# Snoworday/instance-segmentation-attention

Hardware: AMD Instinct MI355X
Metric: images/sec @256x256 bs=16 per GPU (higher is better)
Workload: dtype bf16; 1 GPU; train.py step fwd+bwd+update 256x256 bs=16/GPU (bf16); global_batch=16, parallelism=dp1, launch=hipGraph replay

## Files before the change

include/isa_kernels.h:

```cpp
#ifndef ISA_KERNELS_H
#define ISA_KERNELS_H

#include <stdint.h>

#ifdef __cplusplus
extern "C" {
#endif

enum { ISA_F32 = 0, ISA_BF16 = 1,
       ISA_F16 = 2 };
enum { ISA_ACT_NONE = 0, ISA_ACT_RELU = 1, ISA_ACT_RELU6 = 2, ISA_ACT_LEAKY = 3, ISA_ACT_TANH = 4 };
enum { ISA_STAT_REPLICAS = 8 };
enum { ISA_OK = 0, ISA_EINVAL = -1, ISA_EALIGN = -2, ISA_EDTYPE = -3, ISA_ELAUNCH = -4, ISA_ENOMEM = -5 };

enum { ISA_IN_1X1 = 0,
       ISA_IN_3X3 = 1,
       ISA_IN_GATHER2 = 2 };
enum { ISA_OUT_PLAIN = 0,
       ISA_OUT_SHUFFLE2 = 1 };

typedef struct isa_tensor {
    void*   data;
    int32_t n, h, w;
    int32_t c;
// ... 114 lines not shown
    float count; int32_t c;
} isa_bn_upd;
int isa_bn_running_update(const isa_bn_upd* upd, int32_t n, float momentum, void* stream);
int isa_bn_bwd_reduce(const isa_tensor* dt, const isa_tensor* y, const float* scale,
                      const float* shift, const float* mean, const float* invstd, int32_t act,
                      const float* bscale, float* red, void* stream);
int isa_bn_bwd_apply(const isa_tensor* dt, const isa_tensor* y, const float* scale,
                     const float* shift, const float* mean, const float* invstd, int32_t act,
                     const float* bscale, const float* gamma, const float* red, float count,
                     int32_t train, const isa_tensor* dy, float* dgamma, float* dbeta,
                     void* stream);

int isa_affine_act_res(const isa_tensor* x, const isa_pro* pro, const isa_tensor* res,
                       const isa_tensor* res2, const float* oscale, const isa_tensor* out,
                       void* stream);
int isa_axpy(const isa_tensor* src, const isa_tensor* dst, float alpha, int32_t accumulate,
             void* stream);

int isa_avgpool2(const isa_tensor* x, const isa_tensor* y, void* stream);
int isa_avgpool2_bwd(const isa_tensor* dy, const isa_tensor* dx, int32_t accumulate, void* stream);
int isa_avgpool3(const isa_tensor* x, const isa_tensor* mask, const isa_tensor* y, int32_t accumulate,
                 void* stream);

int isa_chan_mean(const isa_tensor* x, const isa_pro* pro, float* out, void* stream);
int isa_se_fc(const float* mean, const float* w1, const float* b1, const float* w2,
              const float* b2, int32_t n, int32_t c, int32_t hidden, float* hid, float* gate,
              void* stream);
int isa_chan_argmax(const isa_tensor* x, const isa_tensor* y, void* stream);

int isa_mask_dot(const isa_tensor* x, const float* m, const float* w, const float* bias,
// ... 266 lines not shown
```

instance-segmentation-attention_amd/csrc/dwconv.hip:

```cpp
#include "common.hpp"
#include <type_traits>

namespace {

constexpr int TH = 8, TW = 32, CB = 32, PS = 36;
constexpr int HALO = (TH + 2) * (TW + 2);

struct Dw2Params {
    const void* x; const void* w; const float* bias; void* y; const void* dy;
    int n, h, w_, c, ldx, ldy, ldd, wld;
    ProDev pro;
    float* stats; int accumulate;
    int tiles_x, tiles_y; long ntiles;
    float* ws; int csrc;
    int G;
    FinDev fin;
};


struct ProRegs { float sc[8], sh[8], bs[8]; };

template <bool HAS_PRO>
__device__ __forceinline__ void load_pro(const Dw2Params& p, ProRegs& r, int c0, int b) {
#pragma unroll
// ... 514 lines not shown
}

template <typename T>
int launch_fwd2(Dw2Params& p, bool has_pro, hipStream_t s) {
    p.tiles_x = (p.w_ + TW - 1) / TW; p.tiles_y = (p.h + TH - 1) / TH;
    p.ntiles = (long)p.n * p.tiles_x * p.tiles_y;
    if (p.ntiles * p.G >= (1L << 31)) return ISA_EINVAL;
    const int ncb = (p.c + CB - 1) / CB;
    long gx = (256L * (sizeof(T) == 2 ? 1 : 3)) / ncb;
    if (gx < 1) gx = 1;
    if (gx > p.ntiles * p.G) gx = p.ntiles * p.G;
    gx = group_grid(gx, p.G);
    dim3 grid((unsigned)gx, ncb);
    if (p.accumulate) return has_pro ? ISA_EINVAL : launch_fwd2_inst<T, false, ISA_ACT_NONE, true>(p, grid, s);
    if (has_pro && p.pro.act == ISA_ACT_RELU6) return launch_fwd2_inst<T, true, ISA_ACT_RELU6>(p, grid, s);
    if (has_pro) return launch_fwd2_inst<T, true, ACT_RT>(p, grid, s);
    return launch_fwd2_inst<T, false, ISA_ACT_NONE>(p, grid, s);
}

template <typename T>
int launch_wg2(Dw2Params& p, bool has_pro, long ws_floats, isa_slab_arena* sa, const isa_pro* fin, hipStream_t s) {
    p.tiles_x = (p.w_ + TW - 1) / TW; p.tiles_y = (p.h + TH - 1) / TH;
    p.ntiles = (long)p.n * p.tiles_x * p.tiles_y;
    const int ncb = (p.c + CB - 1) / CB;
    long gx = (256L * 2) / ncb;
    if (gx < 1) gx = 1;
    if (gx > p.ntiles * p.G) gx = p.ntiles * p.G;
    if (int rc = defer_ws(sa, &p.ws, &ws_floats)) return rc;
    const long ws_cap = ws_floats / (10L * CB * ncb);
    if (ws_cap < p.G) return sa ? ISA_ENOMEM : ISA_EINVAL;
// ... 21 lines not shown
    int accumulate, tiles_x, tiles_y; long ntiles; float* ws; int csrc; float* dw;
    const void* addend; int lda;
    int G;
};


template <typename T> struct dd_stride { static constexpr int v = 36; };
template <> struct dd_stride<bf16_t> { static constexpr int v = 40; };

constexpr int DW_BIAS = 4;
template <typename T, int YACT, int XMODE_, bool DB, bool EPI>
__global__ __launch_bounds__(DB ? 512 : 256) __attribute__((amdgpu_waves_per_eu(2, 2))) void dw_bn_bwd_kernel(FusedParams p) {
    constexpr int XMODE = XMODE_ & 3;
    constexpr bool BIAS = (XMODE_ & DW_BIAS) != 0;
    constexpr int PSD = dd_stride<T>::v;
    constexpr int XACT = XMODE == 1 ? ISA_ACT_RELU6 : (XMODE == 0 ? ISA_ACT_NONE : ACT_RT);
    constexpr int NBUF = DB ? 2 : 1;
    constexpr int NTHR = DB ? 512 : 256;
    constexpr int TILE_ELEMS = HALO * PSD;
    extern __shared__ __attribute__((aligned(16))) float sm[];
    T* xt_base = reinterpret_cast<T*>(sm);
    T* dt_base = xt_base + NBUF * TILE_ELEMS;
    float* wts = reinterpret_cast<float*>(dt_base + NBUF * TILE_ELEMS);
    float* cst = wts + 9 * CB;
    float* red = cst + 10 * CB;
    f32x4* dbl = reinterpret_cast<f32x4*>(red + 12 * CB);
    constexpr bool DB_LDS = BIAS && XMODE != 0;
    const int tid = threadIdx.x;
    const int ltid = tid & 255;
    const bool loader = DB && tid >= 256;
    const int c_base = blockIdx.y * CB;
// ... 6 lines not shown
        p.ysc += gc; p.ysh += gc; p.ymu += gc; p.yis += gc; p.yred += gc * ISA_STAT_R * 2;
        p.xsc = goff(p.xsc, gc); p.xsh = goff(p.xsh, gc); p.xmu = goff(p.xmu, gc); p.xis = goff(p.xis, gc);
        p.xred = goff(p.xred, gc * ISA_STAT_R * 2);
    }
    const int cg = ltid & 3, g4 = ltid >> 2, row = g4 >> 3, x0 = (g4 & 7) * 4;
    const int c0 = c_base + cg * 8;
    const bool cok = c0 < p.c;
    const T* wp = reinterpret_cast<const T*>(p.w);
    const T* gin = reinterpret_cast<const T*>(p.g);
    const T* yin = reinterpret_cast<const T*>(p.y);
    const T* xin = reinterpret_cast<const T*>(p.x);
    T* dxo = reinterpret_cast<T*>(p.dx);
    constexpr int NIT = (HALO * 4 + 255) / 256;
    constexpr int NB = 3;
    static_assert(NIT % NB == 0, "staging chunks");
    const bool want_xred = XMODE == 1 || (XMODE == 2 && p.xred != nullptr);

    int hrc[NIT], hog[NIT], hoy[NIT], hox[NIT];
    bool hok[NIT];
#pragma unroll
    for (int it = 0; it < NIT; ++it) {
        const int pix = (ltid + it * 256) >> 2;
        const int rr = pix / (TW + 2), cc = pix - rr * (TW + 2);
        const int cc0 = cok ? c0 : c_base;
        hrc[it] = (rr << 16) | cc;
        hog[it] = (rr * p.w_ + cc) * p.ldg + cc0;
        hoy[it] = (rr * p.w_ + cc) * p.ldy + cc0;
        hox[it] = (rr * p.w_ + cc) * p.ldx + cc0;
        hok[it] = pix < HALO && cok;
    }
    const int oodx = (row * p.w_ + x0) * p.lddx + c0, ooa = (row * p.w_ + x0) * p.lda + c0;
// ... 120 lines not shown
    }
    auto compute = [&](int b, int ty, int tx, const T* xt, const T* dt, float (&acc)[9][8], float (&s0)[8], float (&s1)[8]) {
        const long torg = ((long)b * p.h + ty * TH) * p.w_ + tx * TW;
        T* dxb = dxo + torg * p.lddx + oodx;
        const T* adb = reinterpret_cast<const T*>(p.addend) + torg * p.lda + ooa;
        const bool rowok = ty * TH + row < p.h && cok;
        const int xlim = p.w_ - tx * TW;
        raw8<T> oc[4], ad[4];
        if constexpr (EPI) {
            if (rowok) {
#pragma unroll
                for (int o = 0; o < 4; ++o) {
                    if (x0 + o >= xlim) continue;
                    if (p.accumulate) oc[o].load(dxb + o * p.lddx);
                    if constexpr (XMODE == 0) { if (p.addend) ad[o].load(adb + o * p.lda); }
                }
            }
        }
        {
            float a[4][8];
#pragma unroll
            for (int o = 0; o < 4; ++o)
#pragma unroll
                for (int j = 0; j < 8; ++j) a[o][j] = 0.f;
#pragma unroll 1
            for (int dy = 0; dy < 3; ++dy) {
                float wr[3][8], in[6][8];
#pragma unroll
                for (int k = 0; k < 3; ++k) ld8(wts + (dy * 3 + k) * CB + cg * 8, wr[k]);
#pragma unroll
// ... 3 lines not shown
#pragma unroll
                    for (int k = 0; k < 3; ++k)
                        fma8(in[o + k], wr[k], a[o]);
            }
            if (rowok) {
                float xs[8], xh[8], xm[8], xi[8];
                if (want_xred) {
                    ld8(cst + 6 * CB + cg * 8, xs); ld8(cst + 7 * CB + cg * 8, xh);
                    ld8(cst + 8 * CB + cg * 8, xm); ld8(cst + 9 * CB + cg * 8, xi);
                }
#pragma unroll
                for (int o = 0; o < 4; ++o) {
                    if (x0 + o >= xlim) continue;
                    T* dst = dxb + o * p.lddx;
                    if constexpr (EPI) {
                        if (p.accumulate) {
#pragma unroll
                            for (int j = 0; j < 8; ++j) a[o][j] += oc[o].get(j);
                        }
                        if constexpr (XMODE == 0) {
                            if (p.addend) {
#pragma unroll
                                for (int j = 0; j < 8; ++j) a[o][j] += ad[o].get(j);
                            }
                        }
                    }
                    store8<T>(dst, a[o]);
                    if (want_xred) {
                        float xr[8];
                        load8<T>(xt + ((row + 1) * (TW + 2) + x0 + 1 + o) * PSD + cg * 8, xr);
#pragma unroll
// ... 206 lines not shown
    if (gx < 1) gx = 1;
    if (gx > p.ntiles * p.G) gx = p.ntiles * p.G;
    if (int rc = defer_ws(sa, &p.ws, &ws_floats)) return rc;
    const long ws_cap = ws_floats / (10L * CB * ncb);
    if (ws_cap < p.G) return sa ? ISA_ENOMEM : ISA_EINVAL;
    if (gx > ws_cap) gx = ws_cap;
    gx = group_grid(gx, p.G);
    dim3 grid((unsigned)gx, ncb);
    int rc = fin_standalone(xfin, p.c, xfin_groups, s);
    if (rc != ISA_OK) return rc;
    const bool y6 = p.yact == ISA_ACT_RELU6;
#define DW_X(XM) (dbias ? (y6 ? launch_fused_inst<T, ISA_ACT_RELU6, XM, true>(p, grid, s) : launch_fused_inst<T, ACT_RT, XM, true>(p, grid, s)) \
                        : (y6 ? launch_fused_inst<T, ISA_ACT_RELU6, XM, false>(p, grid, s) : launch_fused_inst<T, ACT_RT, XM, false>(p, grid, s)))
    if (xmode == 0) rc = DW_X(0);
    else if (xmode == 1) rc = DW_X(1);
    else rc = DW_X(2);
#undef DW_X
    if (rc != ISA_OK) return rc;
    if (defer_push(sa, FoldDesc{p.ws, p.dw, dbias, nullptr, 1, (int)gx, ncb, 9, 1, 0, CB, p.c, 0, p.csrc, 0, 0, 0, 0},
                   gx * ncb * 10L * CB)) return ISA_OK;
    hipLaunchKernelGGL(dw2_wgrad_reduce_kernel, dim3(ncb, DW2_RSPLIT), dim3(256), 0, s, p.ws, (int)gx, ncb, p.c, p.csrc, p.dw, dbias);
    return launch_status();
}

int dw_forward(const isa_tensor* x, const isa_pro* pro, const void* w, const float* bias, const isa_tensor* y,
               float* stats, int accumulate, void* stream) {
    if (!tensor_ok(x, 8) || !tensor_ok(y, 8) || !w || x->dtype != y->dtype) return ISA_EINVAL;
    if (x->n != y->n || x->h != y->h || x->w != y->w || x->c != y->c) return ISA_EINVAL;
    Dw2Params p{};
    p.x = x->data; p.w = w; p.bias = bias; p.y = y->data;
// ... 66 lines not shown
    if (xp.bscale) return ISA_EINVAL;
    if (xbn && (!xbn->mean || !xbn->invstd || !xbn->out_red)) return ISA_EINVAL;
    FusedParams p{};
    p.g = g->data; p.y = y->data; p.x = x->data; p.w = w_flipped; p.dx = dx->data;
    p.n = g->n; p.h = g->h; p.w_ = g->w; p.c = g->c; p.ldg = g->ld; p.ldy = y->ld; p.ldx = x->ld; p.lddx = dx->ld;
    p.wld = ((g->c + 7) / 8) * 8;
    p.ysc = ybn->scale; p.ysh = ybn->shift; p.ymu = ybn->mean; p.yis = ybn->invstd; p.yred = ybn->red;
    p.ycnt_inv = 1.f / ybn->count; p.yact = ybn->act; p.ydgamma = ybn->dgamma; p.ydbeta = ybn->dbeta;
    p.xsc = xp.scale; p.xsh = xp.shift; p.xact = xp.act;
    p.xmu = xbn ? xbn->mean : nullptr; p.xis = xbn ? xbn->invstd : nullptr; p.xred = xbn ? xbn->out_red : nullptr;
    p.accumulate = accumulate; p.ws = ws; p.dw = dw;
    if (addend) {
        if (!tensor_ok(addend, 8) || addend->dtype != g->dtype || addend->c != g->c || addend->n != g->n || addend->h != g->h ||
            addend->w != g->w) return ISA_EINVAL;
        p.addend = addend->data; p.lda = addend->ld;
        if (!pro_trivial(make_pro(xpro)) || xbn) return ISA_EINVAL;
    }
    p.csrc = (csrc > 0 && csrc < g->c) ? csrc : g->c;
    p.G = tensor_groups(g);
    if (g->n % p.G) return ISA_EINVAL;
    p.n = g->n / p.G;
    int xmode = 0;
    if (!pro_trivial(xp) || xbn) xmode = (xbn && xp.act == ISA_ACT_RELU6) ? 1 : 2;
    if (g->dtype == ISA_BF16) return launch_fused<bf16_t>(p, dbias, xmode, ws_floats, defer, xpro, tensor_groups(x), as_stream(stream));
    return launch_fused<float>(p, dbias, xmode, ws_floats, defer, xpro, tensor_groups(x), as_stream(stream));
}

extern "C" int isa_dwconv3x3_bn_backward(const isa_tensor* g, const isa_tensor* y, const isa_bn_bwd* ybn,
                                         const isa_tensor* x, const isa_pro* xpro, const isa_bn_bwd* xbn,
                                         const void* w_flipped, float* dw, int32_t csrc,
                                         const isa_tensor* dx, int32_t accumulate, const isa_tensor* addend,
                                         float* ws, int64_t ws_floats, isa_slab_arena* defer, void* stream) {
    return isa_dwconv3x3_bias_bn_backward(g, y, ybn, x, xpro, xbn, w_flipped, dw, csrc, dx, accumulate, addend, ws, ws_floats,
                                          defer, stream, nullptr);
}
```

instance-segmentation-attention_amd/csrc/elementwise.hip:

```cpp
#include "common.hpp"

namespace {

template <typename T>
__global__ void pack_kernel(const isa_pack_entry* tab, const int32_t* kmap, const float* src, T* dst) {
    const isa_pack_entry e = tab[blockIdx.y];
    const float* s = src + e.src_off;
    T* d = dst + e.dst_off;
    const int32_t* km = e.kmap_off >= 0 ? kmap + e.kmap_off : nullptr;
    long total;
    const int rows = e.rows;
    switch (e.kind) {
        case 0: case 1: total = (long)rows * e.taps * e.kp; break;
        case 2: total = (long)rows * e.kp; break;
        case 3: total = (long)rows * 4 * e.kp; break;
        default: total = (long)9 * rows; break;
    }
    for (long i = (long)blockIdx.x * blockDim.x + threadIdx.x; i < total; i += (long)gridDim.x * blockDim.x) {
        float v = 0.f;
        if (e.kind == 0) {
            const int kd = (int)(i % e.kp); long q = i / e.kp;
            const int t = (int)(q % e.taps); const int n = (int)(q / e.taps);
            const int k = km ? km[kd] : (kd < e.k ? kd : -1);
            if (k >= 0) v = s[((long)n * e.k + k) * e.taps + t];
// ... 200 lines not shown
                    if (j < nv) { atomicAdd(&red[c0 + j], s0[j]); atomicAdd(&red[C + c0 + j], s1[j]); }
            }
        }
    }
    if (!APPLY) {
        __syncthreads();
        float* rep = p.out_red + (blockIdx.x & (ISA_STAT_R - 1)) * 2 * C;
        for (int i = threadIdx.x; i < 2 * C; i += 256)
            if (red[i] != 0.f) atomicAdd(rep + i, red[i]);
    }
}

struct MatParams { View x, res, res2, out; ProDev pro; const float* oscale; long pixels; int cg; int has_res, has_res2; int groups, bcast; FinDev fin; };
template <typename T, int ACT, bool PI>
__global__ __launch_bounds__(256) STREAM_WAVES(sizeof(T) == 2 ? 5 : 4) void materialize_kernel(MatParams p, Walk wk) {
    const int C = p.x.c;
    __shared__ float fin_tab[2 * ISA_FIN_MAX_C];
    const bool fin = bn_fin_inline<256>(p.fin, C, p.bcast ? 1 : p.groups, p.bcast ? 0 : (int)blockIdx.z, fin_tab, ISA_FIN_MAX_C,
                                        threadIdx.x);
    if (p.groups > 1 && blockIdx.z) {
        const long g = blockIdx.z, gp = g * wk.pixels;
        const long gimg = g * (wk.pixels / ((long)p.x.h * p.x.w)) * C;
        p.out.data = reinterpret_cast<T*>(p.out.data) + gp * p.out.ld;
        if (p.has_res2) p.res2.data = reinterpret_cast<T*>(p.res2.data) + gp * p.res2.ld;
        p.oscale = goff(p.oscale, gimg);
        if (!p.bcast) {
            p.x.data = reinterpret_cast<T*>(p.x.data) + gp * p.x.ld;
            if (p.has_res) p.res.data = reinterpret_cast<T*>(p.res.data) + gp * p.res.ld;
            p.pro.scale = goff(p.pro.scale, g * C); p.pro.shift = goff(p.pro.shift, g * C);
            p.pro.bscale = goff(p.pro.bscale, gimg);
        }
    }
    const int ppb = 256 >> wk.sh;
    const int psub = threadIdx.x >> wk.sh;
    const unsigned hw = (unsigned)p.x.h * (unsigned)p.x.w;
    for (int cgi = threadIdx.x & ((1 << wk.sh) - 1); cgi < wk.cg; cgi += (1 << wk.sh)) {
        const int c0 = cgi * 8;
        const int nv = min(8, C - c0);
        float sc[8], sh[8];
#pragma unroll
        for (int j = 0; j < 8; ++j) {
            const int c = min(c0 + j, C - 1);
            sc[j] = fin ? fin_tab[c] : (p.pro.scale ? p.pro.scale[c] : 1.f);
            sh[j] = fin ? fin_tab[ISA_FIN_MAX_C + c] : (p.pro.shift ? p.pro.shift[c] : 0.f);
        }
        const long step = (long)gridDim.x * ppb;
        const long pix_first = (long)blockIdx.x * ppb + psub;
        float bsr[8], osr[8];
        unsigned bimg = 0;
        auto load_rows = [&](unsigned img) {
            bimg = img;
            const long bofs = (long)img * C + c0;
            if (p.pro.bscale) load_row8(p.pro.bscale + bofs, bsr, nv);
            if (p.oscale) load_row8(p.oscale + bofs, osr, nv);
        };
        if (PI && pix_first < wk.pixels) load_rows((unsigned)pix_first / hw);
        constexpr int U = PI ? 1 : stream_u<T>(STREAM_U_MAT);
        for (long pix0 = pix_first; pix0 < wk.pixels; pix0 += U * step) {
            raw8<T> rx[U], rr[U], rr2[U], rout[U];
            unsigned pixu[U]; bool ok[U];
#pragma unroll
            for (int u = 0; u < U; ++u) {
                const long pix = pix0 + u * step;
                ok[u] = pix < wk.pixels;
                pixu[u] = (unsigned)(ok[u] ? pix : pix0);
            }
#pragma unroll
            for (int u = 0; u < U; ++u) rx[u] = load8raw<T>(reinterpret_cast<const T*>(p.x.data) + (long)pixu[u] * p.x.ld + c0);
            if (p.has_res) {
#pragma unroll
                for (int u = 0; u < U; ++u) rr[u] = load8raw<T>(reinterpret_cast<const T*>(p.res.data) + (long)pixu[u] * p.res.ld + c0);
            }
            if (p.has_res2) {
#pragma unroll
                for (int u = 0; u < U; ++u) rr2[u] = load8raw<T>(reinterpret_cast<const T*>(p.res2.data) + (long)pixu[u] * p.res2.ld + c0);
            }
            __builtin_amdgcn_sched_barrier(0);
#pragma unroll
            for (int u = 0; u < U; ++u) {
                float v[8];
                unpack8m<T>(rx[u], v, nv);
                if (PI) {
                    const unsigned img = pixu[u] / hw;
                    if (img != bimg) load_rows(img);
                }
#pragma unroll
                for (int j = 0; j < 8; ++j) v[j] = act_t<ACT>(fmaf(v[j], sc[j], sh[j]), p.pro.act);
                if (PI && p.pro.bscale) {
#pragma unroll
                    for (int j = 0; j < 8; ++j) v[j] *= bsr[j];
                }
                if (p.has_res) {
                    float r[8];
                    unpack8m<T>(rr[u], r, nv);
#pragma unroll
                    for (int j = 0; j < 8; ++j) v[j] += r[j];
                }
                if (p.has_res2) {
                    float r[8];
                    unpack8m<T>(rr2[u], r, nv);
#pragma unroll
                    for (int j = 0; j < 8; ++j) v[j] += r[j];
                }
                if (PI && p.oscale) {
#pragma unroll
                    for (int j = 0; j < 8; ++j) v[j] *= osr[j];
                }
                rout[u].pack(v);
            }
#pragma unroll
            for (int u = 0; u < U; ++u)
                store8raw<T>(reinterpret_cast<T*>(p.out.data) + (long)pixu[u] * p.out.ld + c0, rout[u], nv);
        }
    }
}

struct AxpyParams { View src, dst; float alpha; int accumulate; long pixels; };
template <typename T>
__global__ __launch_bounds__(256) void axpy_kernel(AxpyParams p) {
    const int C = p.src.c;
    const long items = p.pixels * C;
    for (long i = (long)blockIdx.x * 256 + threadIdx.x; i < items; i += (long)gridDim.x * 256) {
        const int c = (int)(i % C); const long pix = i / C;
        float v = p.alpha == 0.f ? 0.f : p.alpha * st<T>::ld(reinterpret_cast<const T*>(p.src.data) + pix * p.src.ld + c);
        T* d = reinterpret_cast<T*>(p.dst.data) + pix * p.dst.ld + c;
        if (p.accumulate) v += st<T>::ld(d);
        st<T>::stv(d, v);
    }
}
// ... 346 lines not shown
}

extern "C" int isa_bn_bwd_apply(const isa_tensor* dt, const isa_tensor* y, const float* scale,
                                const float* shift, const float* mean, const float* invstd,
                                int32_t act, const float* bscale, const float* gamma,
                                const float* red, float count, int32_t train,
                                const isa_tensor* dy, float* dgamma, float* dbeta, void* stream) {
    if (train && !red) return ISA_EINVAL;
    BnBwdParams p{};
    p.scale = scale; p.shift = shift; p.mean = mean; p.invstd = invstd; p.bscale = bscale;
    p.gamma = gamma; p.red = red; p.inv_count = count > 0 ? 1.f / count : 0.f;
    p.act = act; p.train = train; p.dgamma = dgamma; p.dbeta = dbeta;
    return bn_bwd_common(dt, y, dy, p, true, stream);
}

extern "C" int isa_affine_act_res(const isa_tensor* x, const isa_pro* pro, const isa_tensor* res,
                                  const isa_tensor* res2, const float* oscale,
                                  const isa_tensor* out, void* stream) {
    if (!tensor_ok(x, 8) || !tensor_ok(out, 8)) return ISA_EINVAL;
    const int G = tensor_groups(out);
    const bool bcast = G > 1 && out->n == G * x->n && tensor_groups(x) == 1;
    if (bcast) {
        if (x->h != out->h || x->w != out->w || x->c != out->c || x->dtype != out->dtype) return ISA_EINVAL;
    } else if (!same_shape(x, out)) return ISA_EINVAL;
    if (out->n % G) return ISA_EINVAL;
    if (res && (!tensor_ok(res, 8) || !same_shape(res, x))) return ISA_EINVAL;
    if (res2 && (!tensor_ok(res2, 8) || !same_shape(res2, out))) return ISA_EINVAL;
    MatParams p{};
    p.x = mkview(x); p.out = mkview(out); p.pro = make_pro(pro); p.has_res = res != nullptr;
    p.has_res2 = res2 != nullptr; p.oscale = oscale;
    if (res) p.res = mkview(res);
    if (res2) p.res2 = mkview(res2);
    p.groups = G; p.bcast = bcast;
    p.pixels = (long)(out->n / G) * x->h * x->w; p.cg = (x->c + 7) / 8;
    if (p.pixels * G >= (1L << 32)) return ISA_EINVAL;
    if (pro && pro->fin) {
        if (!fin_valid(pro) || (!bcast && tensor_groups(x) != G)) return ISA_EINVAL;
        if (x->c <= ISA_FIN_MAX_C) p.fin = make_fin(pro);
        else if (int rc = fin_standalone(pro, x->c, tensor_groups(x), as_stream(stream))) return rc;
    }
    const Walk wk = mkwalk(x->c, p.pixels);
    const dim3 grid(walk_grid(wk), 1, G);
    const bool pi = p.pro.bscale || p.oscale;
    by_dtype(x->dtype, [&](auto t) { by_flag(p.pro.act == ISA_ACT_NONE, [&](auto none) { by_flag(pi, [&](auto scaled) {
        constexpr int ACTV = decltype(none)::value ? (int)ISA_ACT_NONE : ACT_RT;
        hipLaunchKernelGGL((materialize_kernel<decltype(t), ACTV, decltype(scaled)::value>), grid, dim3(256), 0, as_stream(stream), p, wk);
    }); }); });
    return launch_status();
}

extern "C" int isa_axpy(const isa_tensor* src, const isa_tensor* dst, float alpha,
                        int32_t accumulate, void* stream) {
    if (!tensor_ok(src, 1) || !tensor_ok(dst, 1) || !same_shape(src, dst)) return ISA_EINVAL;
    AxpyParams p{mkview(src), mkview(dst), alpha, accumulate, (long)src->n * src->h * src->w};
    const bool vec = tensor_ok(src, 8) && tensor_ok(dst, 8) && src->c % 8 == 0;
    const int grid = grid_cap(cdiv(p.pixels * (vec ? src->c / 8 : src->c), 256));
    if (vec)
        by_dtype(src->dtype, [&](auto t) {
            hipLaunchKernelGGL(axpy8_kernel<decltype(t)>, dim3(grid), dim3(256), 0, as_stream(stream), p);
        });
    else
        by_dtype(src->dtype, [&](auto t) {
            hipLaunchKernelGGL(axpy_kernel<decltype(t)>, dim3(grid), dim3(256), 0, as_stream(stream), p);
// ... 108 lines not shown
```

instance-segmentation-attention_amd/engine.py:

```python
import contextlib
import ctypes as C
import os
from typing import Dict, List, Optional, Tuple

import torch

from . import lib as L


STAT_R = 8


def rup(x, m):
    return (x + m - 1) // m * m


class PendingFin:
    __slots__ = ("eng", "stats", "count", "pre", "c", "scale", "shift", "mean", "invstd", "groups", "rep", "running_taken",
                 "done", "keep")

    def __init__(self, eng, stats, count, pre, c, scale, shift, mean, invstd, groups, rep, running_taken):
        self.eng, self.stats, self.count, self.pre, self.c = eng, stats, count, pre, c
        self.scale, self.shift, self.mean, self.invstd, self.groups, self.rep = scale, shift, mean, invstd, groups, rep
        self.running_taken = running_taken
# ... 475 lines not shown
        self.tape = Tape(self)
        self.cur = 0
        self.side_streams: Dict[int, torch.cuda.Stream] = {}
        self.main_stream = None
        self.defer_bn_running = False
        self.bn_running_queue: List[tuple] = []
        self.bn_train = False
        self.record = False
        self.lib = _ProfiledLib(L.checked(), self)
        self.ws = torch.empty(16 << 20, dtype=torch.float32, device=device)
        self.profile = False
        self.prof_events = []
        self.next_bytes = 0
        self.fuse_dw_bn = os.environ.get("ISA_FUSE_DW_BN", "1") != "0"
        self._dw_out: Dict[tuple, ConvFusion] = {}
        self.fuse_pw_bn = os.environ.get("ISA_FUSE_PW_BN", "1") != "0"
        self.pw_recompute = os.environ.get("ISA_PW_RECOMPUTE", "1") != "0"
        self.fuse_bias = os.environ.get("ISA_FUSE_BIAS", "1") != "0"
        self.fuse_eval = os.environ.get("ISA_FUSE_EVAL", "1") != "0"
        self.fuse_block = os.environ.get("ISA_FUSE_BLOCK", "1") != "0"
        self.inline_fin = os.environ.get("ISA_INLINE_FIN", "1") != "0"
        self._pw_out: Dict[tuple, ConvFusion] = {}
        self._pw_in: Dict[tuple, ConvFusion] = {}
        self.eval_bn_cache: Dict[str, tuple] = {}
        self.eval_bn_stale = False
        self.fold_arena = None
        self.slab = None
        self.fold_stats = (0, 0)
        self._deferring = False
        self.defer_fold = os.environ.get("ISA_DEFER_FOLD", "1") != "0"
# ... 334 lines not shown

    def dwconv(self, x: Act, wname, out: Act, *, bias=None, stats=False, kmap=None):
        reg = self.reg_dw(wname, kmap)
        if self.packer.table is None:
            self.packer.pack()
        st = self.scratch(2 * out.c * STAT_R * out.groups) if stats else None
        if self.profile:
            self.next_bytes = 2 * x.n * x.h * x.w * x.c * x.buf.element_size()
        self.lib.isa_dwconv3x3(x.d(), x.p_fin(), self.packer.ptr(reg["fwd"]), self.params.ptr(bias) if bias else None,
                               out.d(), st, self.st())
        if self.record:
            rec = None
            if self.fuse_dw_bn and self.bn_train and x.c % 8 == 0 and (bias is None or self.fuse_bias) and x.needs_grad \
                    and (x.pro is None or x.pro.bscale is None):
                rec = self._dw_out[self._key(out)] = ConvFusion(self._bn_just_recorded(x))
                if x.pro is None and x.bn is None:
                    self._pw_in.setdefault(self._key(x), rec)

            def bwd():
                dy = self.grads.grad_of(out)
                nb = x.n * x.h * x.w * x.c * x.buf.element_size()
                if rec is not None:
                    rec.done = True
                    if rec.ybn is not None:
                        ydesc, xdesc = self._fused_descs(x, rec)
                        acc = self.grads.claim(x, self)
                        if self.profile:
                            self.next_bytes = 4 * nb
                        args = (dy.d(), rec.ybn.raw.d(), C.byref(ydesc), x.d(), x.p(),
                                C.byref(xdesc) if xdesc is not None else None, self.packer.ptr(reg["dgrad"]),
                                self.params.gptr(wname), self.params.shapes[wname][0], self.grads.grad_of(x).d(), acc,
                                rec.addend.d() if rec.addend is not None else None, self.ws, self.ws.numel(),
                                self.defer_handle(), self.st())
                        if bias:
                            self.lib.isa_dwconv3x3_bias_bn_backward(*args, self.params.gptr(bias))
                        else:
                            self.lib.isa_dwconv3x3_bn_backward(*args)
                        return
                    self._flush_addend(x, rec)
                if self.profile:
                    self.next_bytes = 2 * nb
                self.lib.isa_dwconv3x3_wgrad(x.d(), x.p(), dy.d(), self.params.gptr(wname),
                                             self.params.gptr(bias) if bias else None, self.params.shapes[wname][0],
                                             self.ws, self.ws.numel(), self.defer_handle(), self.st())
                if x.needs_grad:
                    acc = self.grads.claim(x, self)
                    if self.profile:
# ... 52 lines not shown
            return red
        if self.profile:
            self.next_bytes = 3 * nb
        self.lib.isa_bn_bwd_apply(dt.d(), b.raw.d(), b.scale, b.shift, b.mean, b.invstd, b.act, bscale,
                                  P.ptr(b.pre + ".weight"), red, b.count, 1 if b.train else 0, dy.d(),
                                  P.gptr(b.pre + ".weight"), P.gptr(b.pre + ".bias"), self.st())
        return red

    def bn_out(self, raw: Act, stats, pre, act, out: Act, res: Optional[Act] = None, bscale=None,
               count=None, res2: Optional[Act] = None, oscale=None) -> Act:
        b, fin = self._bn_layer(raw, stats, pre, act, count)
        lazy = raw.with_pro(Pro(b.scale, b.shift, act, bscale, fin=fin))
        lazy.bn = b
        if self.profile:
            self.next_bytes = (2 + (res is not None) + (res2 is not None)) * raw.n * raw.h * raw.w * raw.c * raw.buf.element_size()
        self.lib.isa_affine_act_res(lazy.d(), lazy.p_fin(), res.d() if res is not None else None,
                                    res2.d() if res2 is not None else None, oscale, out.d(), self.st())
        if self.record:
            pw = self._pw_out.get(self._key(raw)) if (b.train and bscale is None) else None

            bcast = out.n != raw.n
            assert not bcast or (oscale is not None and res2 is None and out.n == out.groups * raw.n and raw.groups == 1)

            def bwd():
                dout = self.grads.grad_of(out)
                dsum = dout
                if oscale is not None:
                    dsum = self.like(raw, out.c)
                    self.lib.isa_scale_bc(dout.d(), oscale, dsum.d(), 0, self.st())
                for r in (res, res2):
                    if r is not None and r.needs_grad:
                        pin = self._pw_in.get(self._key(r))
                        if pin is not None and not pin.done and pin.addend is None:
                            pin.addend = dsum
# ... 83 lines not shown
```

instance-segmentation-attention_amd/lib.py:

```python
import ctypes as C
import os

import torch

_HERE = os.path.dirname(os.path.abspath(__file__))
LIB_PATH = os.environ.get("ISA_KERNELS_LIB") or os.path.join(_HERE, "libisa_kernels.so")

F32, BF16, F16 = 0, 1, 2
ACT_NONE, ACT_RELU, ACT_RELU6, ACT_LEAKY, ACT_TANH = 0, 1, 2, 3, 4
IN_1X1, IN_3X3, IN_GATHER2 = 0, 1, 2
OUT_PLAIN, OUT_SHUFFLE2 = 0, 1
PLANES_U8_NHWK, PLANES_I64_NKHW, PLANES_F32_NKHW = 0, 1, 2
HIST_AGGREGATE, HIST_NAIVE = 0, 1
SEGSORT_TILE = 2048
CC_SPLIT, CC_LARGEST = 0, 1
CC_TILE_H, CC_TILE_W, CC_TAB_BYTES = 32, 64, 4608


def segsort_table_elems(nseg, seglen):
    tiles = (seglen + SEGSORT_TILE - 1) // SEGSORT_TILE
    return nseg * (256 * tiles + (tiles + 7) // 8)


def cc_label_scratch_bytes(n, h, w):
# ... 131 lines not shown
    "isa_rotate_bilinear_u8": [VP, I32, I32, I32, I32, VP, I32, I32, VP, VP, VP],
    "isa_cover_rows_u8": [VP, I32, I32, I32, I32, VP, VP, VP],
    "isa_plane_sums_u8": [VP, I32, I32, I32, I32, I32, I32, I32, I32, VP, VP],
    "isa_crop_planes_u8": [VP, I32, I32, I32, I32, I32, I32, VP, I32, I32, I32, VP, VP],
    "isa_resize_nearest_u8": [VP, I32, I32, I32, I32, VP, I32, I32, VP],
    "isa_resize_bilinear_u8": [VP, I32, I32, I32, I32, VP, I32, I32, VP, I64, VP],
    "isa_resize_lanczos_ws_bytes": [I32, I32, I32, I32, I32, I32, C.POINTER(C.c_int64)],
    "isa_resize_lanczos_u8": [VP, I32, I32, I32, I32, VP, I32, I32, VP, I64, VP],
    "isa_photometric_u8": [VP, VP, I32, I32, I32, VP, I32, VP, VP],
    "isa_collate_targets": [VP, VP, I32, I32, I32, I32, VP, VP, VP],
    "isa_collate_targets_k": [VP, VP, I32, I32, I32, I32, I32, VP, VP, VP, VP],
    "isa_bn_finalize": [VP, F, VP, VP, VP, VP, F, F, VP, VP, VP, VP, I32, I32, I32, VP],
    "isa_bn_bwd_reduce": [P_T, P_T, VP, VP, VP, VP, I32, VP, VP, VP],
    "isa_bn_bwd_apply": [P_T, P_T, VP, VP, VP, VP, I32, VP, VP, VP, F, I32, P_T, VP, VP, VP],
    "isa_affine_act_res": [P_T, P_PRO, P_T, P_T, VP, P_T, VP],
    "isa_axpy": [P_T, P_T, F, I32, VP],
    "isa_avgpool2": [P_T, P_T, VP],
    "isa_avgpool2_bwd": [P_T, P_T, I32, VP],
    "isa_avgpool3": [P_T, P_T, P_T, I32, VP],
    "isa_chan_mean": [P_T, P_PRO, VP, VP],
    "isa_se_fc": [VP, VP, VP, VP, VP, I32, I32, I32, VP, VP, VP],
    "isa_chan_argmax": [P_T, P_T, VP],
    "isa_mask_dot": [P_T, VP, VP, VP, VP, VP, VP],
    "isa_sp_softmax": [VP, VP, VP, VP, VP, VP, I32, I32, I64, VP, VP, VP, VP],
    "isa_scaled_stats": [P_T, VP, VP, VP],
    "isa_sp_apply": [P_T, VP, VP, VP, VP, P_T, VP],
    "isa_maskbn_stats": [P_T, VP, VP, VP, VP],
    "isa_maskbn_finalize": [VP, VP, I32, I32, VP, VP, VP, F, I32, VP],
    "isa_maskbn_apply_pool": [P_T, VP, VP, VP, VP, F, VP, VP],
    "isa_ins_softmax": [VP, VP, VP, I32, I32, I64, VP, VP, I32, VP, VP],
# ... 157 lines not shown
```

instance-segmentation-attention_amd/network.py:

```python
import torch

from . import lib as L
from .engine import Act, Engine, Pro, rup


CRITERIA = ("CE", "Dice", "Multi", "Lovasz", "CELovasz")
LOVASZ_SCRATCH_BYTES = 256 << 20


def lovasz_class_group(K, pixels, backward):
    fixed = 4 * K * pixels if backward else 0
    return max(1, min(K, (LOVASZ_SCRATCH_BYTES - fixed) // (25 * pixels)))


class SemCriterion:

    def __init__(self, n_classes, device):
        self.K = n_classes
        self.cfg = torch.zeros(4 + n_classes, dtype=torch.float32, device=device)
        self.border = torch.tensor([0.0, 5.0], dtype=torch.float32, device=device)
        self.border_on, self.border_weight, self.border_sigma = False, 0.0, 5.0
        self.set("Multi", None, False)

    def set(self, criterion="Multi", class_weights=None, optimize_bg=False, lovasz_per_image=False,
# ... 80 lines not shown
        self.weight = float(weight)
        self.cfg[8:9].fill_(float(weight))

    def key(self):
        return (True, self.form, self.norm) if self.on else (False, None, None)


class Network:
    def __init__(self, eng: Engine, use_instance_seg=True, n_classes=2):
        self.E = eng
        self.use_instance_seg = use_instance_seg
        self.n_classes = n_classes
        self.crit = SemCriterion(n_classes, eng.device)
        self.disc = DiscCriterion(eng.device)

    def block_v1(self, x: Act, pre: str, out: Act):
        E = self.E
        cin = x.c
        cout = E.params.shapes[pre + ".conv.3.weight"][0]
        if E.block_v1_eval_fusable(x, cout):
            return E.block_v1_eval(x, pre, out, res=x if cin == cout else None)
        y1 = E.like(x, cin)
        if E.eval_fusable():
            E.dwconv(x, pre + ".conv.0.weight", y1, stats=False)
            y1 = E.bn(y1, None, pre + ".conv.1", L.ACT_RELU6)
            return E.conv_bn_eval(y1, pre + ".conv.3.weight", out, pre + ".conv.4", L.ACT_NONE, res=x if cin == cout else None)
        _, s1 = E.dwconv(x, pre + ".conv.0.weight", y1, stats=True)
        y1 = E.bn(y1, s1, pre + ".conv.1", L.ACT_RELU6)
        y2 = E.like(x, cout)
        _, s2 = E.conv(y1, pre + ".conv.3.weight", y2, stats=True)
        return E.bn_out(y2, s2, pre + ".conv.4", L.ACT_NONE, out, res=x if cin == cout else None)

    def block_ir(self, x: Act, pre: str, out: Act, oscale=None):
        E = self.E
# ... 8 lines not shown
            y2 = E.bn(y2, None, pre + ".conv.4", L.ACT_RELU6)
            return E.conv_bn_eval(y2, pre + ".conv.6.weight", out, pre + ".conv.7", L.ACT_NONE, res=x if cin == cout else None)
        _, s1 = E.conv(x, pre + ".conv.0.weight", y1, stats=True)
        y1 = E.bn(y1, s1, pre + ".conv.1", L.ACT_RELU6)
        y2 = E.like(x, chid)
        _, s2 = E.dwconv(y1, pre + ".conv.3.weight", y2, stats=True)
        y2 = E.bn(y2, s2, pre + ".conv.4", L.ACT_RELU6)
        y3 = E.like(x, cout)
        _, s3 = E.conv(y2, pre + ".conv.6.weight", y3, stats=True)
        return E.bn_out(y3, s3, pre + ".conv.7", L.ACT_NONE, out, res=x if cin == cout else None,
                        oscale=oscale)

    def double_v1(self, x: Act, pre: str, out: Act):
        E = self.E
        cmid = E.params.shapes[pre + ".conv.down_conv_0.conv.3.weight"][0]
        mid = E.like(x, cmid)
        self.block_v1(x, pre + ".conv.down_conv_0", mid)
        return self.block_v1(mid, pre + ".conv.down_conv_1", out)

    def unet(self, x_in: Act):
        E = self.E
        n, h, w = x_in.n, x_in.h, x_in.w
        widths = [(64, 32), (128, 64), (256, 128), (512, 256), (512, 512)]
        bufs = []
        for lvl, (ld, _) in enumerate(widths):
            bufs.append(E.new_act(n, h >> lvl, w >> lvl, ld, ld=ld))
        x1 = bufs[0].slice(0, 32)
        self.double_v1(x_in, "base.inc.conv", x1)
        feats = [x1]
        cur = x1
        for lvl in range(1, 5):
            cw = widths[lvl][1] // 2
# ... 400 lines not shown
```

Measured before the change: 759.9 images/s.

## Keep double-conv mid activation lazy and fold its BN into consumers

In double_v1 blocks where the channel count changes, the first block's output BN (no activation) is no longer written out as a materialized tensor. It stays lazy, so the next depthwise conv applies the affine in its prologue, and the residual materialize kernel applies it to the residual read. The depthwise BN backward gains a mode (XMODE 3) for a lazy BN input with no activation, including addend accumulation. This removes one full activation write and read per block pair, at the cost of more kernel template variants and an extra axpy on some backward paths.

```diff
diff --git a/include/isa_kernels.h b/include/isa_kernels.h
--- a/include/isa_kernels.h
+++ b/include/isa_kernels.h
@@ -152,6 +152,9 @@
 int isa_affine_act_res(const isa_tensor* x, const isa_pro* pro, const isa_tensor* res,
                        const isa_tensor* res2, const float* oscale, const isa_tensor* out,
                        void* stream);
+int isa_affine_act_res_pro(const isa_tensor* x, const isa_pro* pro, const isa_tensor* res, const isa_pro* res_pro,
+                           const isa_tensor* res2, const float* oscale, const isa_tensor* out,
+                           void* stream);
 int isa_axpy(const isa_tensor* src, const isa_tensor* dst, float alpha, int32_t accumulate,
              void* stream);
 
diff --git a/instance-segmentation-attention_amd/csrc/dwconv.hip b/instance-segmentation-attention_amd/csrc/dwconv.hip
--- a/instance-segmentation-attention_amd/csrc/dwconv.hip
+++ b/instance-segmentation-attention_amd/csrc/dwconv.hip
@@ -5,6 +5,10 @@
 
 constexpr int TH = 8, TW = 32, CB = 32, PS = 36;
 constexpr int HALO = (TH + 2) * (TW + 2);
+
+#ifndef ISA_DW_AFFINE_CT
+#define ISA_DW_AFFINE_CT 1
+#endif
 
 struct Dw2Params {
     const void* x; const void* w; const float* bias; void* y; const void* dy;
@@ -552,6 +556,7 @@
     dim3 grid((unsigned)gx, ncb);
     if (p.accumulate) return has_pro ? ISA_EINVAL : launch_fwd2_inst<T, false, ISA_ACT_NONE, true>(p, grid, s);
     if (has_pro && p.pro.act == ISA_ACT_RELU6) return launch_fwd2_inst<T, true, ISA_ACT_RELU6>(p, grid, s);
+    if (ISA_DW_AFFINE_CT && has_pro && p.pro.act == ISA_ACT_NONE) return launch_fwd2_inst<T, true, ISA_ACT_NONE>(p, grid, s);
     if (has_pro) return launch_fwd2_inst<T, true, ACT_RT>(p, grid, s);
     return launch_fwd2_inst<T, false, ISA_ACT_NONE>(p, grid, s);
 }
@@ -603,7 +608,7 @@
     constexpr int XMODE = XMODE_ & 3;
     constexpr bool BIAS = (XMODE_ & DW_BIAS) != 0;
     constexpr int PSD = dd_stride<T>::v;
-    constexpr int XACT = XMODE == 1 ? ISA_ACT_RELU6 : (XMODE == 0 ? ISA_ACT_NONE : ACT_RT);
+    constexpr int XACT = XMODE == 1 ? ISA_ACT_RELU6 : ((XMODE == 0 || XMODE == 3) ? ISA_ACT_NONE : ACT_RT);
     constexpr int NBUF = DB ? 2 : 1;
     constexpr int NTHR = DB ? 512 : 256;
     constexpr int TILE_ELEMS = HALO * PSD;
@@ -640,7 +645,7 @@
     constexpr int NIT = (HALO * 4 + 255) / 256;
     constexpr int NB = 3;
     static_assert(NIT % NB == 0, "staging chunks");
-    const bool want_xred = XMODE == 1 || (XMODE == 2 && p.xred != nullptr);
+    const bool want_xred = XMODE == 1 || XMODE == 3 || (XMODE == 2 && p.xred != nullptr);
 
     int hrc[NIT], hog[NIT], hoy[NIT], hox[NIT];
     bool hok[NIT];
@@ -791,6 +796,7 @@
                     if (x0 + o >= xlim) continue;
                     if (p.accumulate) oc[o].load(dxb + o * p.lddx);
                     if constexpr (XMODE == 0) { if (p.addend) ad[o].load(adb + o * p.lda); }
+                    else { if (p.addend) oc[o].load(adb + o * p.lda); }
                 }
             }
         }
@@ -824,7 +830,7 @@
                     if (x0 + o >= xlim) continue;
                     T* dst = dxb + o * p.lddx;
                     if constexpr (EPI) {
-                        if (p.accumulate) {
+                        if (p.accumulate || (XMODE != 0 && p.addend)) {
 #pragma unroll
                             for (int j = 0; j < 8; ++j) a[o][j] += oc[o].get(j);
                         }
@@ -1061,6 +1067,7 @@
                         : (y6 ? launch_fused_inst<T, ISA_ACT_RELU6, XM, false>(p, grid, s) : launch_fused_inst<T, ACT_RT, XM, false>(p, grid, s)))
     if (xmode == 0) rc = DW_X(0);
     else if (xmode == 1) rc = DW_X(1);
+    else if (xmode == 3) rc = DW_X(3);
     else rc = DW_X(2);
 #undef DW_X
     if (rc != ISA_OK) return rc;
@@ -1157,14 +1164,14 @@
         if (!tensor_ok(addend, 8) || addend->dtype != g->dtype || addend->c != g->c || addend->n != g->n || addend->h != g->h ||
             addend->w != g->w) return ISA_EINVAL;
         p.addend = addend->data; p.lda = addend->ld;
-        if (!pro_trivial(make_pro(xpro)) || xbn) return ISA_EINVAL;
+        if ((!pro_trivial(xp) || xbn) && accumulate) return ISA_EINVAL;
     }
     p.csrc = (csrc > 0 && csrc < g->c) ? csrc : g->c;
     p.G = tensor_groups(g);
     if (g->n % p.G) return ISA_EINVAL;
     p.n = g->n / p.G;
     int xmode = 0;
-    if (!pro_trivial(xp) || xbn) xmode = (xbn && xp.act == ISA_ACT_RELU6) ? 1 : 2;
+    if (!pro_trivial(xp) || xbn) xmode = (xbn && xp.act == ISA_ACT_RELU6) ? 1 : ((ISA_DW_AFFINE_CT && xbn && xp.act == ISA_ACT_NONE) ? 3 : 2);
     if (g->dtype == ISA_BF16) return launch_fused<bf16_t>(p, dbias, xmode, ws_floats, defer, xpro, tensor_groups(x), as_stream(stream));
     return launch_fused<float>(p, dbias, xmode, ws_floats, defer, xpro, tensor_groups(x), as_stream(stream));
 }
diff --git a/instance-segmentation-attention_amd/csrc/elementwise.hip b/instance-segmentation-attention_amd/csrc/elementwise.hip
--- a/instance-segmentation-attention_amd/csrc/elementwise.hip
+++ b/instance-segmentation-attention_amd/csrc/elementwise.hip
@@ -238,105 +238,15 @@
 struct MatParams { View x, res, res2, out; ProDev pro; const float* oscale; long pixels; int cg; int has_res, has_res2; int groups, bcast; FinDev fin; };
 template <typename T, int ACT, bool PI>
 __global__ __launch_bounds__(256) STREAM_WAVES(sizeof(T) == 2 ? 5 : 4) void materialize_kernel(MatParams p, Walk wk) {
-    const int C = p.x.c;
-    __shared__ float fin_tab[2 * ISA_FIN_MAX_C];
-    const bool fin = bn_fin_inline<256>(p.fin, C, p.bcast ? 1 : p.groups, p.bcast ? 0 : (int)blockIdx.z, fin_tab, ISA_FIN_MAX_C,
-                                        threadIdx.x);
-    if (p.groups > 1 && blockIdx.z) {
-        const long g = blockIdx.z, gp = g * wk.pixels;
-        const long gimg = g * (wk.pixels / ((long)p.x.h * p.x.w)) * C;
-        p.out.data = reinterpret_cast<T*>(p.out.data) + gp * p.out.ld;
-        if (p.has_res2) p.res2.data = reinterpret_cast<T*>(p.res2.data) + gp * p.res2.ld;
-        p.oscale = goff(p.oscale, gimg);
-        if (!p.bcast) {
-            p.x.data = reinterpret_cast<T*>(p.x.data) + gp * p.x.ld;
-            if (p.has_res) p.res.data = reinterpret_cast<T*>(p.res.data) + gp * p.res.ld;
-            p.pro.scale = goff(p.pro.scale, g * C); p.pro.shift = goff(p.pro.shift, g * C);
-            p.pro.bscale = goff(p.pro.bscale, gimg);
-        }
-    }
-    const int ppb = 256 >> wk.sh;
-    const int psub = threadIdx.x >> wk.sh;
-    const unsigned hw = (unsigned)p.x.h * (unsigned)p.x.w;
-    for (int cgi = threadIdx.x & ((1 << wk.sh) - 1); cgi < wk.cg; cgi += (1 << wk.sh)) {
-        const int c0 = cgi * 8;
-        const int nv = min(8, C - c0);
-        float sc[8], sh[8];
-#pragma unroll
-        for (int j = 0; j < 8; ++j) {
-            const int c = min(c0 + j, C - 1);
-            sc[j] = fin ? fin_tab[c] : (p.pro.scale ? p.pro.scale[c] : 1.f);
-            sh[j] = fin ? fin_tab[ISA_FIN_MAX_C + c] : (p.pro.shift ? p.pro.shift[c] : 0.f);
-        }
-        const long step = (long)gridDim.x * ppb;
-        const long pix_first = (long)blockIdx.x * ppb + psub;
-        float bsr[8], osr[8];
-        unsigned bimg = 0;
-        auto load_rows = [&](unsigned img) {
-            bimg = img;
-            const long bofs = (long)img * C + c0;
-            if (p.pro.bscale) load_row8(p.pro.bscale + bofs, bsr, nv);
-            if (p.oscale) load_row8(p.oscale + bofs, osr, nv);
-        };
-        if (PI && pix_first < wk.pixels) load_rows((unsigned)pix_first / hw);
-        constexpr int U = PI ? 1 : stream_u<T>(STREAM_U_MAT);
-        for (long pix0 = pix_first; pix0 < wk.pixels; pix0 += U * step) {
-            raw8<T> rx[U], rr[U], rr2[U], rout[U];
-            unsigned pixu[U]; bool ok[U];
-#pragma unroll
-            for (int u = 0; u < U; ++u) {
-                const long pix = pix0 + u * step;
-                ok[u] = pix < wk.pixels;
-                pixu[u] = (unsigned)(ok[u] ? pix : pix0);
-            }
-#pragma unroll
-            for (int u = 0; u < U; ++u) rx[u] = load8raw<T>(reinterpret_cast<const T*>(p.x.data) + (long)pixu[u] * p.x.ld + c0);
-            if (p.has_res) {
-#pragma unroll
-                for (int u = 0; u < U; ++u) rr[u] = load8raw<T>(reinterpret_cast<const T*>(p.res.data) + (long)pixu[u] * p.res.ld + c0);
-            }
-            if (p.has_res2) {
-#pragma unroll
-                for (int u = 0; u < U; ++u) rr2[u] = load8raw<T>(reinterpret_cast<const T*>(p.res2.data) + (long)pixu[u] * p.res2.ld + c0);
-            }
-            __builtin_amdgcn_sched_barrier(0);
-#pragma unroll
-            for (int u = 0; u < U; ++u) {
-                float v[8];
-                unpack8m<T>(rx[u], v, nv);
-                if (PI) {
-                    const unsigned img = pixu[u] / hw;
-                    if (img != bimg) load_rows(img);
-                }
-#pragma unroll
-                for (int j = 0; j < 8; ++j) v[j] = act_t<ACT>(fmaf(v[j], sc[j], sh[j]), p.pro.act);
-                if (PI && p.pro.bscale) {
-#pragma unroll
-                    for (int j = 0; j < 8; ++j) v[j] *= bsr[j];
-                }
-                if (p.has_res) {
-                    float r[8];
-                    unpack8m<T>(rr[u], r, nv);
-#pragma unroll
-                    for (int j = 0; j < 8; ++j) v[j] += r[j];
-                }
-                if (p.has_res2) {
-                    float r[8];
-                    unpack8m<T>(rr2[u], r, nv);
-#pragma unroll
-                    for (int j = 0; j < 8; ++j) v[j] += r[j];
-                }
-                if (PI && p.oscale) {
-#pragma unroll
-                    for (int j = 0; j < 8; ++j) v[j] *= osr[j];
-                }
-                rout[u].pack(v);
-            }
-#pragma unroll
-            for (int u = 0; u < U; ++u)
-                store8raw<T>(reinterpret_cast<T*>(p.out.data) + (long)pixu[u] * p.out.ld + c0, rout[u], nv);
-        }
-    }
+    constexpr bool RP = false;
+    constexpr int RACT = ISA_ACT_NONE;
+    ProDev rp{};
+#include "materialize_body.inc"
+}
+template <typename T, int ACT, bool PI, int RACT>
+__global__ __launch_bounds__(256) STREAM_WAVES((sizeof(T) == 2 && !PI) ? 5 : 4) void materialize_rp_kernel(MatParams p, ProDev rp, Walk wk) {
+    constexpr bool RP = true;
+#include "materialize_body.inc"
 }
 
 struct AxpyParams { View src, dst; float alpha; int accumulate; long pixels; };
@@ -713,10 +623,14 @@
     return bn_bwd_common(dt, y, dy, p, true, stream);
 }
 
-extern "C" int isa_affine_act_res(const isa_tensor* x, const isa_pro* pro, const isa_tensor* res,
-                                  const isa_tensor* res2, const float* oscale,
-                                  const isa_tensor* out, void* stream) {
+extern "C" int isa_affine_act_res_pro(const isa_tensor* x, const isa_pro* pro, const isa_tensor* res, const isa_pro* res_pro,
+                                      const isa_tensor* res2, const float* oscale,
+                                      const isa_tensor* out, void* stream) {
     if (!tensor_ok(x, 8) || !tensor_ok(out, 8)) return ISA_EINVAL;
+    const ProDev rp = make_pro(res_pro);
+    if (res_pro && (res_pro->bscale || res_pro->fin)) return ISA_EINVAL;
+    const bool lazy_res = !pro_trivial(rp);
+    if (lazy_res && !res) return ISA_EINVAL;
     const int G = tensor_groups(out);
     const bool bcast = G > 1 && out->n == G * x->n && tensor_groups(x) == 1;
     if (bcast) {
@@ -743,9 +657,23 @@
     const bool pi = p.pro.bscale || p.oscale;
     by_dtype(x->dtype, [&](auto t) { by_flag(p.pro.act == ISA_ACT_NONE, [&](auto none) { by_flag(pi, [&](auto scaled) {
         constexpr int ACTV = decltype(none)::value ? (int)ISA_ACT_NONE : ACT_RT;
-        hipLaunchKernelGGL((materialize_kernel<decltype(t), ACTV, decltype(scaled)::value>), grid, dim3(256), 0, as_stream(stream), p, wk);
+        if (!lazy_res) {
+            hipLaunchKernelGGL((materialize_kernel<decltype(t), ACTV, decltype(scaled)::value>), grid, dim3(256), 0, as_stream(stream), p, wk);
+            return;
+        }
+        by_flag(rp.act == ISA_ACT_NONE, [&](auto rnone) {
+            constexpr int RACTV = decltype(rnone)::value ? (int)ISA_ACT_NONE : ACT_RT;
+            hipLaunchKernelGGL((materialize_rp_kernel<decltype(t), ACTV, decltype(scaled)::value, RACTV>), grid, dim3(256), 0,
+                               as_stream(stream), p, rp, wk);
+        });
     }); }); });
     return launch_status();
+}
+
+extern "C" int isa_affine_act_res(const isa_tensor* x, const isa_pro* pro, const isa_tensor* res,
+                                  const isa_tensor* res2, const float* oscale,
+                                  const isa_tensor* out, void* stream) {
+    return isa_affine_act_res_pro(x, pro, res, nullptr, res2, oscale, out, stream);
 }
 
 extern "C" int isa_axpy(const isa_tensor* src, const isa_tensor* dst, float alpha,
diff --git a/instance-segmentation-attention_amd/csrc/materialize_body.inc b/instance-segmentation-attention_amd/csrc/materialize_body.inc
--- /dev/null
+++ b/instance-segmentation-attention_amd/csrc/materialize_body.inc
@@ -0,0 +1,111 @@
+    const int C = p.x.c;
+    __shared__ float fin_tab[2 * ISA_FIN_MAX_C];
+    const bool fin = bn_fin_inline<256>(p.fin, C, p.bcast ? 1 : p.groups, p.bcast ? 0 : (int)blockIdx.z, fin_tab, ISA_FIN_MAX_C,
+                                        threadIdx.x);
+    if (p.groups > 1 && blockIdx.z) {
+        const long g = blockIdx.z, gp = g * wk.pixels;
+        const long gimg = g * (wk.pixels / ((long)p.x.h * p.x.w)) * C;
+        p.out.data = reinterpret_cast<T*>(p.out.data) + gp * p.out.ld;
+        if (p.has_res2) p.res2.data = reinterpret_cast<T*>(p.res2.data) + gp * p.res2.ld;
+        p.oscale = goff(p.oscale, gimg);
+        if (!p.bcast) {
+            p.x.data = reinterpret_cast<T*>(p.x.data) + gp * p.x.ld;
+            if (p.has_res) p.res.data = reinterpret_cast<T*>(p.res.data) + gp * p.res.ld;
+            p.pro.scale = goff(p.pro.scale, g * C); p.pro.shift = goff(p.pro.shift, g * C);
+            p.pro.bscale = goff(p.pro.bscale, gimg);
+            if constexpr (RP) { rp.scale = goff(rp.scale, g * C); rp.shift = goff(rp.shift, g * C); }
+        }
+    }
+    const int ppb = 256 >> wk.sh;
+    const int psub = threadIdx.x >> wk.sh;
+    const unsigned hw = (unsigned)p.x.h * (unsigned)p.x.w;
+    for (int cgi = threadIdx.x & ((1 << wk.sh) - 1); cgi < wk.cg; cgi += (1 << wk.sh)) {
+        const int c0 = cgi * 8;
+        const int nv = min(8, C - c0);
+        float sc[8], sh[8];
+        float rsc[8], rsh[8];
+#pragma unroll
+        for (int j = 0; j < 8; ++j) {
+            const int c = min(c0 + j, C - 1);
+            sc[j] = fin ? fin_tab[c] : (p.pro.scale ? p.pro.scale[c] : 1.f);
+            sh[j] = fin ? fin_tab[ISA_FIN_MAX_C + c] : (p.pro.shift ? p.pro.shift[c] : 0.f);
+        }
+        if constexpr (RP) {
+#pragma unroll
+            for (int j = 0; j < 8; ++j) { rsc[j] = 1.f; rsh[j] = 0.f; }
+            if (rp.scale) load_row8(rp.scale + c0, rsc, nv);
+            if (rp.shift) load_row8(rp.shift + c0, rsh, nv);
+        }
+        const long step = (long)gridDim.x * ppb;
+        const long pix_first = (long)blockIdx.x * ppb + psub;
+        float bsr[8], osr[8];
+        unsigned bimg = 0;
+        auto load_rows = [&](unsigned img) {
+            bimg = img;
+            const long bofs = (long)img * C + c0;
+            if (p.pro.bscale) load_row8(p.pro.bscale + bofs, bsr, nv);
+            if (p.oscale) load_row8(p.oscale + bofs, osr, nv);
+        };
+        if (PI && pix_first < wk.pixels) load_rows((unsigned)pix_first / hw);
+        constexpr int U = PI ? 1 : stream_u<T>(STREAM_U_MAT);
+        for (long pix0 = pix_first; pix0 < wk.pixels; pix0 += U * step) {
+            raw8<T> rx[U], rr[U], rr2[U], rout[U];
+            unsigned pixu[U]; bool ok[U];
+#pragma unroll
+            for (int u = 0; u < U; ++u) {
+                const long pix = pix0 + u * step;
+                ok[u] = pix < wk.pixels;
+                pixu[u] = (unsigned)(ok[u] ? pix : pix0);
+            }
+#pragma unroll
+            for (int u = 0; u < U; ++u) rx[u] = load8raw<T>(reinterpret_cast<const T*>(p.x.data) + (long)pixu[u] * p.x.ld + c0);
+            if (p.has_res) {
+#pragma unroll
+                for (int u = 0; u < U; ++u) rr[u] = load8raw<T>(reinterpret_cast<const T*>(p.res.data) + (long)pixu[u] * p.res.ld + c0);
+            }
+            if (p.has_res2) {
+#pragma unroll
+                for (int u = 0; u < U; ++u) rr2[u] = load8raw<T>(reinterpret_cast<const T*>(p.res2.data) + (long)pixu[u] * p.res2.ld + c0);
+            }
+            __builtin_amdgcn_sched_barrier(0);
+#pragma unroll
+            for (int u = 0; u < U; ++u) {
+                float v[8];
+                unpack8m<T>(rx[u], v, nv);
+                if (PI) {
+                    const unsigned img = pixu[u] / hw;
+                    if (img != bimg) load_rows(img);
+                }
+#pragma unroll
+                for (int j = 0; j < 8; ++j) v[j] = act_t<ACT>(fmaf(v[j], sc[j], sh[j]), p.pro.act);
+                if (PI && p.pro.bscale) {
+#pragma unroll
+                    for (int j = 0; j < 8; ++j) v[j] *= bsr[j];
+                }
+                if (p.has_res) {
+                    float r[8];
+                    unpack8m<T>(rr[u], r, nv);
+                    if constexpr (RP) {
+#pragma unroll
+                        for (int j = 0; j < 8; ++j) r[j] = act_t<RACT>(fmaf(r[j], rsc[j], rsh[j]), rp.act);
+                    }
+#pragma unroll
+                    for (int j = 0; j < 8; ++j) v[j] += r[j];
+                }
+                if (p.has_res2) {
+                    float r[8];
+                    unpack8m<T>(rr2[u], r, nv);
+#pragma unroll
+                    for (int j = 0; j < 8; ++j) v[j] += r[j];
+                }
+                if (PI && p.oscale) {
+#pragma unroll
+                    for (int j = 0; j < 8; ++j) v[j] *= osr[j];
+                }
+                rout[u].pack(v);
+            }
+#pragma unroll
+            for (int u = 0; u < U; ++u)
+                store8raw<T>(reinterpret_cast<T*>(p.out.data) + (long)pixu[u] * p.out.ld + c0, rout[u], nv);
+        }
+    }
diff --git a/instance-segmentation-attention_amd/engine.py b/instance-segmentation-attention_amd/engine.py
--- a/instance-segmentation-attention_amd/engine.py
+++ b/instance-segmentation-attention_amd/engine.py
@@ -513,6 +513,7 @@
         self.next_bytes = 0
         self.fuse_dw_bn = os.environ.get("ISA_FUSE_DW_BN", "1") != "0"
         self._dw_out: Dict[tuple, ConvFusion] = {}
+        self.lazy_mid = os.environ.get("ISA_LAZY_MID", "1") != "0"
         self.fuse_pw_bn = os.environ.get("ISA_FUSE_PW_BN", "1") != "0"
         self.pw_recompute = os.environ.get("ISA_PW_RECOMPUTE", "1") != "0"
         self.fuse_bias = os.environ.get("ISA_FUSE_BIAS", "1") != "0"
@@ -877,7 +878,7 @@
             if self.fuse_dw_bn and self.bn_train and x.c % 8 == 0 and (bias is None or self.fuse_bias) and x.needs_grad \
                     and (x.pro is None or x.pro.bscale is None):
                 rec = self._dw_out[self._key(out)] = ConvFusion(self._bn_just_recorded(x))
-                if x.pro is None and x.bn is None:
+                if (x.pro is None and x.bn is None) or (self.lazy_mid and rec.xbn is not None):
                     self._pw_in.setdefault(self._key(x), rec)
 
             def bwd():
@@ -888,12 +889,16 @@
                     if rec.ybn is not None:
                         ydesc, xdesc = self._fused_descs(x, rec)
                         acc = self.grads.claim(x, self)
+                        addend = rec.addend
+                        if addend is not None and acc and (x.pro is not None or xdesc is not None):
+                            self.lib.isa_axpy(addend.d(), self.grads.grad_of(x).d(), 1.0, 1, self.st())
+                            addend = None
                         if self.profile:
                             self.next_bytes = 4 * nb
                         args = (dy.d(), rec.ybn.raw.d(), C.byref(ydesc), x.d(), x.p(),
                                 C.byref(xdesc) if xdesc is not None else None, self.packer.ptr(reg["dgrad"]),
                                 self.params.gptr(wname), self.params.shapes[wname][0], self.grads.grad_of(x).d(), acc,
-                                rec.addend.d() if rec.addend is not None else None, self.ws, self.ws.numel(),
+                                addend.d() if addend is not None else None, self.ws, self.ws.numel(),
                                 self.defer_handle(), self.st())
                         if bias:
                             self.lib.isa_dwconv3x3_bias_bn_backward(*args, self.params.gptr(bias))
@@ -976,10 +981,15 @@
         lazy.bn = b
         if self.profile:
             self.next_bytes = (2 + (res is not None) + (res2 is not None)) * raw.n * raw.h * raw.w * raw.c * raw.buf.element_size()
-        self.lib.isa_affine_act_res(lazy.d(), lazy.p_fin(), res.d() if res is not None else None,
-                                    res2.d() if res2 is not None else None, oscale, out.d(), self.st())
+        if res is not None and res.pro is not None:
+            assert res.pro.bscale is None, "a lazy residual carries scale, shift and act only"
+            self.lib.isa_affine_act_res_pro(lazy.d(), lazy.p_fin(), res.d(), res.p(),
+                                            res2.d() if res2 is not None else None, oscale, out.d(), self.st())
+        else:
+            self.lib.isa_affine_act_res(lazy.d(), lazy.p_fin(), res.d() if res is not None else None,
+                                        res2.d() if res2 is not None else None, oscale, out.d(), self.st())
         if self.record:
-            pw = self._pw_out.get(self._key(raw)) if (b.train and bscale is None) else None
+            pw =self._pw_out.get(self._key(raw)) if (b.train and bscale is None) else None
 
             bcast = out.n != raw.n
             assert not bcast or (oscale is not None and res2 is None and out.n == out.groups * raw.n and raw.groups == 1)
diff --git a/instance-segmentation-attention_amd/lib.py b/instance-segmentation-attention_amd/lib.py
--- a/instance-segmentation-attention_amd/lib.py
+++ b/instance-segmentation-attention_amd/lib.py
@@ -169,6 +169,7 @@
     "isa_bn_bwd_reduce": [P_T, P_T, VP, VP, VP, VP, I32, VP, VP, VP],
     "isa_bn_bwd_apply": [P_T, P_T, VP, VP, VP, VP, I32, VP, VP, VP, F, I32, P_T, VP, VP, VP],
     "isa_affine_act_res": [P_T, P_PRO, P_T, P_T, VP, P_T, VP],
+    "isa_affine_act_res_pro": [P_T, P_PRO, P_T, P_PRO, P_T, VP, P_T, VP],
     "isa_axpy": [P_T, P_T, F, I32, VP],
     "isa_avgpool2": [P_T, P_T, VP],
     "isa_avgpool2_bwd": [P_T, P_T, I32, VP],
diff --git a/instance-segmentation-attention_amd/network.py b/instance-segmentation-attention_amd/network.py
--- a/instance-segmentation-attention_amd/network.py
+++ b/instance-segmentation-attention_amd/network.py
@@ -1,3 +1,5 @@
+from typing import Optional
+
 import torch
 
 from . import lib as L
@@ -118,10 +120,18 @@
         self.crit = SemCriterion(n_classes, eng.device)
         self.disc = DiscCriterion(eng.device)
 
-    def block_v1(self, x: Act, pre: str, out: Act):
+    def block_v1(self, x: Act, pre: str, out: Optional[Act], lazy_out=False):
         E = self.E
         cin = x.c
         cout = E.params.shapes[pre + ".conv.3.weight"][0]
+        if lazy_out:
+            assert E.bn_train and cin != cout
+            y1 = E.like(x, cin)
+            _, s1 = E.dwconv(x, pre + ".conv.0.weight", y1, stats=True)
+            y1 = E.bn(y1, s1, pre + ".conv.1", L.ACT_RELU6)
+            y2 = E.like(x, cout)
+            _, s2 = E.conv(y1, pre + ".conv.3.weight", y2, stats=True)
+            return E.bn(y2, s2, pre + ".conv.4", L.ACT_NONE)
         if E.block_v1_eval_fusable(x, cout):
             return E.block_v1_eval(x, pre, out, res=x if cin == cout else None)
         y1 = E.like(x, cin)
@@ -160,8 +170,11 @@
     def double_v1(self, x: Act, pre: str, out: Act):
         E = self.E
         cmid = E.params.shapes[pre + ".conv.down_conv_0.conv.3.weight"][0]
-        mid = E.like(x, cmid)
-        self.block_v1(x, pre + ".conv.down_conv_0", mid)
+        if E.lazy_mid and E.fuse_dw_bn and E.bn_train and x.c != cmid:
+            mid = self.block_v1(x, pre + ".conv.down_conv_0", None, lazy_out=True)
+        else:
+            mid = E.like(x, cmid)
+            self.block_v1(x, pre + ".conv.down_conv_0", mid)
         return self.block_v1(mid, pre + ".conv.down_conv_1", out)
 
     def unet(self, x_in: Act):
```

Result: no change. 762.3 images/s (median of 4 runs) (+0.3%).
